# razvanmatisan/duodiff

Measured on AMD Instinct MI355X. Metric: images/sec (whole node) DuoDiff 1000-step CelebA-64, higher is better.
Workload: dtype bf16

## Files before the change

duodiff_amd/csrc/dd_internal.h:

```cpp
#pragma once
#include <hip/hip_runtime.h>
#include <stdint.h>

namespace dd {

typedef unsigned short bf16_t;

typedef __attribute__((ext_vector_type(8))) short bf16x8;
typedef __attribute__((ext_vector_type(4))) float f32x4;
typedef __attribute__((ext_vector_type(16))) float f32x16;
typedef unsigned u32x2 __attribute__((ext_vector_type(2)));
typedef unsigned u32x4 __attribute__((ext_vector_type(4)));

__device__ __forceinline__ bf16_t f2bf(float f) {
    __bf16 b = (__bf16)f;
    return __builtin_bit_cast(unsigned short, b);
}
__device__ __forceinline__ float bf2f(bf16_t b) {
    return __builtin_bit_cast(float, ((unsigned)b) << 16);
}

template <typename T> struct Elem;
template <> struct Elem<float> {
    static constexpr int kPerChunk = 4;
// ... 166 lines not shown
    const char* wimg;
    const float* bias;
    float* xres;
    const float *ln_g, *ln_b;
    bf16_t* h_out;
    bf16_t* h_frag;
    bf16_t* x_copy;
    float* partial;
    int M;
    int tok_n, tok_e, tok_l, n_main, n_extra, tiles_main, tiles_extra, groups, cpg;
};
bool rowlin_supported(int D, int K);
void rowlin_pack(int K, const float* w, unsigned short (*to_bf16)(float), unsigned short* img);
void rowlin_plan(int B, int n_patches, int extras, int seq_len, int K, RowLinArgs& a);
size_t rowlin_partial_bytes(int max_batch, int extras, int K);
hipError_t launch_rowlin(const RowLinArgs& a, hipStream_t s);
hipError_t init_rowlin_kernels();

struct EmbedArgs {
    const float* x_img;
    const float* wt;
    const float* bias;
    const float* pos;
    const float* label_emb;
    const long long* y;
    const float* t_vec;
    StepState* st;
    float* x_tok;
    int B, C, S, P, D, L, extras, num_classes, normalize, Mp;
    int generic;
    const float* ln_g = nullptr;
    const float* ln_b = nullptr;
    bf16_t* ln_frag = nullptr;
};
bool embed_ln_supported(const EmbedArgs& a);

struct ReduceLnArgs {
    float* x;
    const float* partial;
    long long slab;
    int splits, resid;
    const float* bias;
    bf16_t* copy;
    int ldo;
    const float *ln_g, *ln_b;
    bf16_t* h;
    bf16_t* frag;
    int tok_l, tok_e;
    int rows;
};
hipError_t launch_reduce_ln(const ReduceLnArgs& a, int D, hipStream_t s);
hipError_t launch_embed(const EmbedArgs& a, hipStream_t s);

struct TimeMlpArgs {
    const float *w1t, *b1, *w2t, *b2, *pos, *t_vec;
    const StepState* st;
    float* x_tok;
    int B, D, L, extras, normalize;
};
hipError_t launch_time_mlp(const TimeMlpArgs& a, hipStream_t s);

template <typename T>
hipError_t launch_layernorm(const float* x, const float* gamma, const float* beta, T* out,
                            int rows, int D, hipStream_t s);
hipError_t launch_layernorm_frag(const float* x, const float* gamma, const float* beta, bf16_t* out, bf16_t* frag, int rows, int D,
                                 int tok_l, int tok_e, hipStream_t s);
// ... 153 lines not shown
```

duodiff_amd/csrc/dev_harness.hip:

```cpp
#include "../../include/duodiff.h"
#include "../../include/duodiff_dev.h"
#include "engine_state.h"
#include "launch_args.h"

#include <cstring>
#include <vector>

using namespace dd;

extern "C" {

int dd_dev_mlp(dd_ctx* c, int M, int D, int hidden, int extras, const float* x_host, const float* w1, const float* b1, const float* w2,
               const float* b2, float* xres_host, unsigned short* out_host, const float* ln_in, const float* ln_out,
               unsigned short* ln_out_host, int iters, void* stream, float* ms_out, const float* ao_host, const float* wproj,
               const float* bproj, const float* skip_host, const float* wskip, const float* bskip, const float* wqkv,
               unsigned short* qkv_out_host) {
    const bool proj = ao_host && wproj && bproj;
    const bool skp = skip_host && wskip && bskip;
    const bool qk = wqkv && qkv_out_host;
    if (qk && (!proj || !ln_out || (hidden / 32) % 2)) return DD_ERR_INVALID;
    if (proj && (!ln_in || D % 128)) return DD_ERR_INVALID;
    if (skp && (!proj || !ln_out || !ln_out_host || (hidden / 32) % 2)) return DD_ERR_INVALID;
    if (!c || !x_host || !w1 || !b1 || !w2 || !b2 || !xres_host || M < 1 || iters < 0 || extras < 0 || (extras > 0 && M % (1 + extras))) return DD_ERR_INVALID;
    if (!mlp_fused_supported(D, hidden)) return ctx_fail(c, DD_ERR_UNSUPPORTED, "fused MLP: D in {64,128,256,512}, hidden % 64 == 0");
// ... 492 lines not shown
    const bool bf = precision == DD_PREC_BF16;
    if (!c || (!bf && precision != DD_PREC_FP32) || rows < 1 || rows > (1 << 24) || D < 64 || D % 64 || D > 4096 || !last_host || !prev_host ||
        !out_host || op < 0 || op > 2 || iters < 0)
        return DD_ERR_INVALID;
    hipStream_t s = (hipStream_t)stream;
    const size_t es = bf ? 2 : 4, n = (size_t)rows * D, n_out = ((size_t)rows + 8) * D;
    DevScope dev(c);
    const void* dL = dev.upload((const char*)last_host, n * es);
    const void* dP = dev.upload((const char*)prev_host, n * es);
    void* dO = dev.filled(n_out * es, 0xFF);
    std::vector<AffineRow> tab(3);
    memset((void*)tab.data(), 0xFF, tab.size() * sizeof(AffineRow));
    tab[1].pad1 = op; tab[1].pad2 = __builtin_bit_cast(int, w);
    const StepState st_host{1, 0.f, 0ull, 1, 0};
    const AffineRow* dT = table ? dev.upload(tab.data(), tab.size() * sizeof(AffineRow)) : nullptr;
    const StepState* dS = table ? dev.upload(&st_host, sizeof(StepState)) : nullptr;
    auto once = [&]() { return launch_cache_extrapolate(dL, dP, dO, (long long)n, bf, dS, dT, table ? -1 : op, table ? __builtin_nanf("") : w, s); };
    DEV_HIP(dev, once());
    DEV_HIP(dev, hipStreamSynchronize(s));
    dev.download(out_host, dO, n_out * es);
    DEV_HIP(dev, time_launches(s, iters, once, ms_out));
    return dev.status();
}

int dd_dev_embed(dd_ctx* c, int B, int C, int S, int P, int D, int extras, int num_classes, int normalize, int generic, const float* x_img,
                 const float* w, const float* bias, const float* pos, const float* label_emb, const long long* y, const float* t_vec,
                 float t_state, const float* ln, float* x_tok_host, unsigned short* ln_frag_host, int iters, void* stream, float* ms_out) {
    if (!c || B < 1 || C < 1 || P < 1 || S < P || S % P || D < 2 || extras < 1 || extras > 2 || !x_img || !w || !bias || !pos || !x_tok_host ||
        (extras == 2 && (!label_emb || !y || num_classes < 1)) || (ln && !ln_frag_host) || iters < 0)
        return DD_ERR_INVALID;
    const int pd = C * P * P, L = extras + (S / P) * (S / P), Mp = round_up(B * L, 256);
    if (pd > 64) return ctx_fail(c, DD_ERR_UNSUPPORTED, "embed: patch_dim <= 64");
    hipStream_t s = (hipStream_t)stream;
    const std::vector<float> wt = transposed(w, D, pd);
    const size_t n_tok = ((size_t)Mp + 8) * D;
    EmbedArgs a{};
    a.B = B; a.C = C; a.S = S; a.P = P; a.D = D; a.L = L; a.extras = extras; a.num_classes = num_classes; a.normalize = normalize; a.Mp = Mp;
    a.generic = generic;
    if (ln && !embed_ln_supported(a)) return ctx_fail(c, DD_ERR_UNSUPPORTED, "embed with norm1: the MFMA kernel at patch 4, 3 channels, embed_dim 512");
    DevScope dev(c);
    a.x_img = dev.upload(x_img, (size_t)B * C * S * S * 4);
    a.wt = dev.upload(wt.data(), wt.size() * 4);
    a.bias = dev.upload(bias, (size_t)D * 4);
    a.pos = dev.upload(pos, (size_t)L * D * 4);
    if (extras == 2) { a.label_emb = dev.upload(label_emb, (size_t)num_classes * D * 4); a.y = dev.upload(y, (size_t)B * 8); }
    if (t_vec) a.t_vec = dev.upload(t_vec, (size_t)B * 4);
    a.st = dev.alloc<StepState>(sizeof(StepState));
    a.x_tok = dev.filled<float>(n_tok * 4, 0xFF);
    if (ln) {
        a.ln_g = dev.upload(ln, (size_t)2 * D * 4); a.ln_b = a.ln_g + D;
        a.ln_frag = dev.filled<bf16_t>(n_tok * 2, 0xFF);
    }
    DEV_HIP(dev, launch_set_state_float(a.st, t_state, s));
    auto once = [&]() { return launch_embed(a, s); };
    DEV_HIP(dev, once());
    DEV_HIP(dev, hipStreamSynchronize(s));
    dev.download(x_tok_host, a.x_tok, n_tok * 4);
    if (ln) dev.download(ln_frag_host, a.ln_frag, n_tok * 2);
    DEV_HIP(dev, time_launches(s, iters, once, ms_out));
    return dev.status();
}

int dd_dev_time_mlp(dd_ctx* c, int B, int D, int L, int extras, int normalize, const float* w1, const float* b1, const float* w2,
                    const float* b2, const float* pos, const float* t_vec, float t_state, float* x_tok_host, int iters, void* stream,
                    float* ms_out) {
    if (!c || B < 1 || D < 2 || extras < 1 || L < extras || !w1 || !b1 || !w2 || !b2 || !pos || !x_tok_host || iters < 0) return DD_ERR_INVALID;
    if ((size_t)5 * D * 4 > 64 * 1024) return ctx_fail(c, DD_ERR_UNSUPPORTED, "time_mlp: 5 D floats of LDS");
    hipStream_t s = (hipStream_t)stream;
    const int H4 = 4 * D;
    const std::vector<float> w1t = transposed(w1, H4, D), w2t = transposed(w2, D, H4);
    const size_t n_tok = (size_t)B * L * D;
    DevScope dev(c);
    StepState* st = dev.alloc<StepState>(sizeof(StepState));
    float* dX = dev.upload(x_tok_host, n_tok * 4);
    const TimeMlpArgs a{dev.upload(w1t.data(), w1t.size() * 4), dev.upload(b1, (size_t)H4 * 4), dev.upload(w2t.data(), w2t.size() * 4),
// ... 421 lines not shown
```

duodiff_amd/csrc/engine_state.h:

```cpp
#pragma once
#include "../../include/duodiff.h"
#include "dd_internal.h"
#include "dev_scope.h"

#include <map>
#include <string>
#include <vector>

#define DD_HIP(c, expr)                                          \
    do {                                                         \
        hipError_t _e = (expr);                                  \
        if (_e != hipSuccess) return dd::fail_hip((c), _e, #expr);   \
    } while (0)

#pragma GCC visibility push(hidden)
namespace dd {
template <typename T>
struct DevBuf {
    T* p = nullptr;
    size_t n = 0;
    int grow(dd_ctx* c, size_t need) {
        if (n >= need) return DD_OK;
        release();
        DD_HIP(c, hipMalloc((void**)&p, need * sizeof(T)));
// ... 114 lines not shown
    bf16_t* qkv_dump = nullptr;
    bf16_t* hfrag = nullptr;
    bf16_t* aofrag = nullptr;
    std::vector<bf16_t*> skipfrags;
    float* xfrag = nullptr;
    float* ytap = nullptr;
};

struct BlockCache {
    void *last = nullptr, *prev = nullptr, *yhat = nullptr;
    int K = 0, rows = 0, b0 = 0, B = 0;
    bool has_last = false, has_prev = false;
    bool holds(int K_, int rows_, int b0_, int B_) const { return has_last && K == K_ && rows == rows_ && b0 == b0_ && B == B_; }
    void refresh(int K_, int rows_, int b0_, int B_, bool rotate) {
        has_prev = rotate && holds(K_, rows_, b0_, B_);
        K = K_; rows = rows_; b0 = b0_; B = B_; has_last = true;
    }
};

}
#pragma GCC visibility pop

struct dd_model {
    dd_ctx* ctx = nullptr;
    unsigned long long serial = 0;
    dd_config cfg{};
    int D = 0, L = 0, N = 0, extras = 0, pd = 0, pdp = 0, H = 0, hidden = 0, hid_ld = 0, half_depth = 0, Mp_max = 0;
    std::map<std::string, dd::HostParam> params;
    bool finalized = false;
    int prec = DD_PREC_BF16;
    size_t esize = 2;
    char* warena = nullptr;
    std::vector<dd::BlockW> blocks;
    const float *emb_wt = nullptr, *emb_b = nullptr, *pos = nullptr, *label = nullptr;
    const float *tm_w1t = nullptr, *tm_b1 = nullptr, *tm_w2t = nullptr, *tm_b2 = nullptr;
    dd::HeadW head{};
    int ee_type = -1, n_probe = 0;
    std::vector<dd::HeadW> heads;
    const float *probe_w = nullptr, *probe_b = nullptr;
    std::vector<dd::AttnProbeW> attn_probes;
    bool ee_conv_stride_ok = false;
    long long ee_wconv_stride = 0, ee_bconv_stride = 0;
    bool ee_batched = false;
    bool fused_mlp = false;
    bool fused_proj = false;
    bool fused_skip = false;
    bool fused_qkv = false;
    bool splitk = false;
    bool rowlin_skip = false;
    bool rowlin_proj = false;
    bool rowlin_fc2 = false;
    bool frag_ao = false;
    bool frag_skip = false;
    bool frag_x = false;
    bool fused_qa = false;
    size_t ws_bytes[2] = {0, 0};
    char* wsarena[2] = {nullptr, nullptr};
    dd::WsPtrs ws[2];
    hipGraphExec_t graph[dd::GRAPH_KINDS][2] = {};
    dd::GraphKey gkey[dd::GRAPH_KINDS][2]{};
    dd::BlockCache cache[2];
    float* ee_ws = nullptr;
    int* real_tabs = nullptr;
    int* real_counts_host = nullptr;
    hipEvent_t real_ev[2] = {nullptr, nullptr};
    bool time_fc1 = false;
    std::vector<hipEvent_t> fc1_events;
// ... 119 lines not shown
```

duodiff_amd/csrc/forward.hip:

```cpp
#include "../../include/duodiff.h"
#include "../../include/duodiff_dev.h"
#include "engine_state.h"
#include "launch_args.h"

#include <cmath>

using namespace dd;

namespace dd {
Mods perturbed(const dd_pag* p, const dd_model* late) {
    Mods mo{};
    mo.pag = p; mo.pag_late = late; mo.missing = p ? nullptr : "null dd_pag";
    return mo;
}

const char* check_threshold(const dd_x0_threshold* t) {
    if (!t) return "null dd_x0_threshold";
    if (t->mode == DD_X0_STATIC) return t->range > 0.f && std::isfinite(t->range) ? nullptr : "dd_x0_threshold: range must be positive and finite";
    if (t->mode != DD_X0_DYNAMIC) return "dd_x0_threshold: unknown mode";
    if (!(t->quantile > 0.f && t->quantile <= 1.f)) return "dd_x0_threshold: quantile outside (0, 1]";
    if (!(t->s_max >= 1.f)) return "dd_x0_threshold: s_max must be at least 1 (it may be +inf)";
    return nullptr;
}
X0Threshold kernel_threshold(const dd_x0_threshold* t, long long n) {
// ... 45 lines not shown
        if (!m->time_fc1 || kind != prof) return DD_OK;
        while (m->fc1_events.size() < m->fc1_used + 1) {
            hipEvent_t e;
            DD_HIP(c, hipEventCreate(&e));
            m->fc1_events.push_back(e);
        }
        DD_HIP(c, hipEventRecord(m->fc1_events[m->fc1_used++], s));
        return DD_OK;
    }
#define DD_TIMED(kind, expr) \
    do { if (int rc_ = mark(kind)) return rc_; DD_HIP(c, expr); if (int rc_ = mark(kind)) return rc_; } while (0)

    int tile128(int N, int K, int K1) const { return bf16 && gemm_prefers_128(m->cfg.max_batch * L, N, K, K1, c->num_cus) ? 1 : 0; }
    const T* skip_of(int bi) const { return (const T*)ws.skips[nb - 1 - bi]; }
    Handoff norm1_written() const { return Handoff{!m->fused_qa, m->fused_qa}; }

    int rowlin_then_reduce(const GemmArgs<bf16_t>& g, int resid, const char* wimg, const float* ln_g, const float* ln_b, bool frag) {
        const RowLinArgs ra = rowlin_args(g, resid, wimg, ws.mlp_partial, ln_g, ln_b, (bf16_t*)h, frag ? ws.hfrag : nullptr, B, m->N, m->extras);
        DD_TIMED(DD_PROF_ROWLIN, launch_rowlin(ra, s));
        DD_HIP(c, launch_mlp_reduce(rowlin_reduce_args(ra), D, s));
        return DD_OK;
    }
    int splitk_then_reduce_ln(GemmArgs<bf16_t> g, int resid, const float* ln_g, const float* ln_b, bool frag) {
        g.partial = ws.mlp_partial; g.splits = 2;
        DD_TIMED(DD_PROF_SPLITK, launch_gemm_splitk(g, s, ch.cus));
        DD_HIP(c, launch_reduce_ln(splitk_reduce_args(g, resid, ln_g, ln_b, (bf16_t*)h, frag ? ws.hfrag : nullptr, L, m->extras), D, s));
        return DD_OK;
    }

    int embed(const float* x_img, const float* t_vec, const int64_t* y_dev, Handoff& first) {
        EmbedArgs ea{x_img, m->emb_wt, m->emb_b, m->pos, m->label, (const long long*)y_dev, t_vec, ch.st, ws.x,
                     B, m->cfg.in_chans, m->cfg.img_size, m->cfg.patch_size, D, L, m->extras,
                     m->cfg.num_classes, m->cfg.normalize_timesteps, round_up(M, 256), (c->dev_flags & DD_DEV_GENERIC_EMBED) ? 1 : 0};
        if constexpr (bf16) {
            if (m->fused_qa && !(c->dev_flags & DD_DEV_NO_EMBED_LN) && embed_ln_supported(ea)) {
                ea.ln_g = m->blocks[0].ln1_g; ea.ln_b = m->blocks[0].ln1_b; ea.ln_frag = ws.hfrag;
                first.frag = true;
            }
        }
        DD_HIP(c, launch_embed(ea, s));
        if (m->tm_w1t) {
            TimeMlpArgs ta{m->tm_w1t, m->tm_b1, m->tm_w2t, m->tm_b2, m->pos, t_vec, ch.st, ws.x, B, D, L, m->extras, m->cfg.normalize_timesteps};
            DD_HIP(c, launch_time_mlp(ta, s));
        }
        return DD_OK;
    }

    int ee_taps(int bi, const Handoff& in, bool& side) {
        if (!ee) return DD_OK;
        const HeadW& hd = m->heads[bi];
        const float* xin = (in.skip && ws.ytap) ? ws.ytap : ws.x;
        side = bi <= m->half_depth && ch.ee_fork && c->side && s != c->side;
        hipStream_t hs = side ? c->side : s;
        if (side) {
            DD_HIP(c, hipEventRecord(c->ev_ee_fork, s));
            DD_HIP(c, hipStreamWaitEvent(c->side, c->ev_ee_fork, 0));
        }
        const int t_mul = m->ee_type == DD_EE_MLP_PER_LAYER ? 0 : m->ee_type == DD_EE_MLP_PER_TIMESTEP ? 1 : nb;
        const int add = m->ee_type == DD_EE_MLP_PER_TIMESTEP ? 0 : bi;
        bool probe_done = false;
        if (hd.wg) {
            HeadDecArgs ha{xin, hd.wg, hd.dc, ee_dec_all ? ee_dec_all + (size_t)bi * Bs * L * m->pd : ws.dec, M, m->pd, (L - m->extras) % 16 == 0 ? L : 0, m->extras};
            if (hd.wsplit) { ha.wg = hd.wsplit; ha.c = hd.dcs; ha.split = 1; }
            if (ee_srow_all && m->ee_type != DD_EE_ATTENTION_PROBE && head_dec_probe_supported(D)) {
                ha.srow = ee_srow_all + (size_t)bi * Bs * L; ha.pw_base = m->probe_w; ha.pb_base = m->probe_b; ha.st = ch.st; ha.t_mul = t_mul; ha.add = add;
                probe_done = true;
// ... 564 lines not shown
```

duodiff_amd/csrc/launch_args.h:

```cpp
#pragma once
#include "dd_internal.h"
#include "host_arena.h"

#include <cmath>
#include <vector>

namespace dd {
#pragma GCC visibility push(hidden)

inline int round_up(int v, int m) { return (v + m - 1) / m * m; }

struct TailImage {
    std::vector<unsigned short> img;
    std::vector<float> b1p;
};
inline TailImage pack_tail_image(int D, int hidden, const float* wproj, const float* w1, const float* b1, const float* w2, bool kperm, const float* wskip,
                                 const float* wqkv) {
    const MlpImage im = MlpImage::of(D, hidden, wproj != nullptr, wskip != nullptr, wqkv != nullptr);
    TailImage t{std::vector<unsigned short>(im.bytes() / 2, 0), std::vector<float>(hidden)};
    auto section = [&](size_t block) { return t.img.data() + im.at(block) / 2; };
    if (wproj) mlp_fused_pack_proj(D, wproj, host_f2bf, section(0));
    mlp_fused_pack(D, hidden, w1, b1, w2, kperm, host_f2bf, section(im.mlp), t.b1p.data());
    if (wskip) mlp_fused_pack_skip(D, wskip, host_f2bf, section(im.skip));
    if (wqkv) mlp_fused_pack_rows(D, 3 * D, wqkv, host_f2bf, section(im.qkv));
    return t;
}

inline std::vector<float> transposed(const float* w, int out, int in) {
    std::vector<float> wt((size_t)in * out);
    for (int o = 0; o < out; ++o) for (int k = 0; k < in; ++k) wt[(size_t)k * out + o] = w[(size_t)o * in + k];
    return wt;
}

struct HeadImage {
    std::vector<float> wg, dc, dcs;
    std::vector<unsigned short> wsplit;
};
inline HeadImage pack_head_image(int D, int pd, const float* wd, const float* bd, const float* ng, const float* nb, bool split) {
    HeadImage h;
    h.wg.assign((size_t)pd * D, 0.f);
    h.dc.assign(2 * (size_t)pd, 0.f);
    for (int r = 0; r < pd; ++r) {
        double acc = bd[r], wsum = 0.0;
        for (int k = 0; k < D; ++k) {
            h.wg[(size_t)r * D + k] = wd[(size_t)r * D + k] * ng[k];
            acc += (double)wd[(size_t)r * D + k] * (double)nb[k];
            wsum += (double)h.wg[(size_t)r * D + k];
        }
        h.dc[r] = (float)acc;
        h.dc[pd + r] = (float)wsum;
    }
    if (split) {
        h.wsplit = std::vector<unsigned short>((size_t)(D / 32) * ((pd + 15) / 16) * 2 * 64 * 8, 0);
        const float* c = h.dc.data();
        h.dcs.assign(c, c + 2 * (size_t)pd);
        pack_head_split(D, pd, h.wg.data(), host_f2bf, h.wsplit.data(), h.dcs.data() + pd);
    }
    return h;
}

struct AttnProbeFold {
    std::vector<float> u, wvt, w0t;
};
inline AttnProbeFold fold_attn_probe(int D, const float* q, const float* wkv, const float* w0) {
// ... 65 lines not shown
```

duodiff_amd/csrc/model.hip:

```cpp
#include "../../include/duodiff.h"
#include "../../include/duodiff_dev.h"
#include "engine_state.h"
#include "host_arena.h"
#include "launch_args.h"

#include <algorithm>
#include <atomic>
#include <cmath>
#include <cstring>
#include <map>
#include <new>
#include <string>
#include <vector>

using namespace dd;

namespace dd {
int ctx_fail(dd_ctx* c, int code, const std::string& msg) {
    if (c) c->err = msg;
    return code;
}
}

namespace {
// ... 163 lines not shown
    auto P = [&](const std::string& n) -> const std::vector<float>& { return param(m, n); };
    BlockW& w = m->blocks[bi];
    a.f32(w.ln1_g, P(p + "norm1.weight")); a.f32(w.ln1_b, P(p + "norm1.bias"));
    a.f32(w.ln2_g, P(p + "norm2.weight")); a.f32(w.ln2_b, P(p + "norm2.bias"));
    a.f32(w.proj_b, P(p + "attn.proj.bias"));
    a.f32(w.fc1_b, P(p + "mlp.fc1.bias")); a.f32(w.fc2_b, P(p + "mlp.fc2.bias"));
    a.mat(w.qkv_w, P(p + "attn.qkv.weight")); a.mat(w.proj_w, P(p + "attn.proj.weight"));
    if (m->cfg.qkv_bias) a.f32(w.qkv_b, P(p + "attn.qkv.bias"));
    a.mat(w.fc1_w, P(p + "mlp.fc1.weight")); a.mat(w.fc2_w, P(p + "mlp.fc2.weight"));
    const bool skip = bi > m->half_depth;
    if (skip) { a.f32(w.skip_b, P(p + "skip_linear.bias")); a.mat(w.skip_w, P(p + "skip_linear.weight")); }
    if (m->fused_mlp) {
        const bool with_skip = m->fused_skip && !next_skip.empty();
        const bool with_qkv = m->fused_qkv && !m->fused_qa && !next_qkv.empty() && (next_skip.empty() || with_skip);
        const TailImage t = pack_tail_image(D, hid, m->fused_proj ? P(p + "attn.proj.weight").data() : nullptr, P(p + "mlp.fc1.weight").data(),
                                            P(p + "mlp.fc1.bias").data(), P(p + "mlp.fc2.weight").data(), true,
                                            with_skip ? P(next_skip + "skip_linear.weight").data() : nullptr,
                                            with_qkv ? P(next_qkv + "attn.qkv.weight").data() : nullptr);
        std::memcpy(a.raw(w.mlp_img, t.img.size() * 2), t.img.data(), t.img.size() * 2);
        a.f32(w.mlp_b1p, t.b1p);
    }
    if (m->fused_qa)
        qkv_attention_pack(D, m->H, P(p + "attn.qkv.weight").data(), host_f2bf, (unsigned short*)a.raw(w.qa_img, (size_t)3 * D * D * 2));
    if (m->rowlin_fc2) {
        rowlin_pack(hid, P(p + "mlp.fc2.weight").data(), host_f2bf, (unsigned short*)a.raw(w.rl_img, (size_t)D * hid * 2));
        rowlin_pack(D, P(p + "attn.proj.weight").data(), host_f2bf, (unsigned short*)a.raw(w.rlp_img, (size_t)D * D * 2));
        if (skip) rowlin_pack(2 * D, P(p + "skip_linear.weight").data(), host_f2bf, (unsigned short*)a.raw(w.rls_img, (size_t)D * 2 * D * 2));
    }
}

void pack_embed(dd_model* m, Arena& a) {
    const int D = m->D, pd = m->pd;
    auto P = [&](const std::string& n) -> const std::vector<float>& { return param(m, n); };
    a.f32(m->emb_wt, transposed(P("patch_embed.proj.weight").data(), D, pd)); a.f32(m->emb_b, P("patch_embed.proj.bias")); a.f32(m->pos, P("pos_embed"));
    if (m->cfg.num_classes > 0) a.f32(m->label, P("label_emb.weight"));
    if (m->cfg.mlp_time_embed) {
        a.f32(m->tm_w1t, transposed(P("time_embed.0.weight").data(), 4 * D, D)); a.f32(m->tm_b1, P("time_embed.0.bias"));
        a.f32(m->tm_w2t, transposed(P("time_embed.2.weight").data(), D, 4 * D)); a.f32(m->tm_b2, P("time_embed.2.bias"));
    }
}

void pack_head(const dd_model* m, Arena& a, const std::string& p, HeadW& h, bool fused, bool split) {
    const int D = m->D, pd = m->pd;
    auto P = [&](const std::string& n) -> const std::vector<float>& { return param(m, n); };
    const std::vector<float>&ng = P(p + "norm.weight"), &nb = P(p + "norm.bias"), &wd = P(p + "decoder_pred.weight"), &bd = P(p + "decoder_pred.bias");
    a.f32(h.ng, ng); a.f32(h.nb, nb); a.f32(h.wdec, wd); a.f32(h.bdec, bd);
    a.f32(h.wconv, P(p + "final_layer.weight")); a.f32(h.bconv, P(p + "final_layer.bias"));
    if (!fused) return;
    const HeadImage hi = pack_head_image(D, pd, wd.data(), bd.data(), ng.data(), nb.data(), split);
    a.f32(h.wg, hi.wg); a.f32(h.dc, hi.dc);
    if (!split) return;
    std::memcpy(a.raw(h.wsplit, hi.wsplit.size() * 2), hi.wsplit.data(), hi.wsplit.size() * 2);
    a.f32(h.dcs, hi.dcs);
}

void pack_probes(dd_model* m, Arena& a) {
    const int D = m->D;
    auto P = [&](const std::string& n) -> const std::vector<float>& { return param(m, n); };
    int nt, nl;
    probe_grid(m, nt, nl);
    if (m->ee_type == DD_EE_ATTENTION_PROBE) {
        m->attn_probes.resize(nl);
        for (int layer = 0; layer < nl; ++layer) {
            const std::string pre = "matrix." + probe_key(m, layer, 0) + ".";
            const std::vector<float>&q = P(pre + "q"), &wkv = P(pre + "weight_kv.weight"), &bkv = P(pre + "weight_kv.bias"),
                                    &w0 = P(pre + "classification.0.weight");
            const AttnProbeFold f = fold_attn_probe(D, q.data(), wkv.data(), w0.data());
// ... 246 lines not shown
```

duodiff_amd/csrc/rowops.hip:

```cpp
#include "dd_internal.h"
#include "wave_prims.h"

#include <cstring>
#include <utility>
#include <vector>

#include <cstdlib>

namespace dd {
namespace {

constexpr int kEmbedTok = 8;

__global__ void __launch_bounds__(256) embed_kernel(const EmbedArgs a) {
    __shared__ float patch[kEmbedTok][64];
    const int rows_per_img_blocks = (a.L + kEmbedTok - 1) / kEmbedTok;
    const int b = blockIdx.x / rows_per_img_blocks;
    const int r0 = (blockIdx.x % rows_per_img_blocks) * kEmbedTok;
    const int tid = threadIdx.x;
    const int pd = a.C * a.P * a.P;
    const int g = a.S / a.P;
    if (blockIdx.x == 0 && tid == 0) a.st->t_final = a.st->t;

    if (b >= a.B) {
// ... 33 lines not shown
#pragma unroll
            for (int j = 0; j < kEmbedTok; ++j) acc[j] = fmaf(w, patch[j][k], acc[j]);
        }
        const float bias = a.bias[d];
#pragma unroll
        for (int j = 0; j < kEmbedTok; ++j) {
            const int row = r0 + j;
            if (row >= a.L) continue;
            float v;
            if (row >= a.extras) {
                v = acc[j] + bias;
            } else if (row == a.extras - 1) {
                const int i = d < halfd ? d : d - halfd;
                const float f = expf((-9.210340371976184f * (float)i) / (float)halfd);
                const float arg = tt * f;
                v = (d < halfd) ? cosf(arg) : (d < 2 * halfd ? sinf(arg) : 0.f);
            } else {
                long long yy = a.y[b];
                yy = yy < 0 ? 0 : (yy >= a.num_classes ? a.num_classes - 1 : yy);
                v = a.label_emb[yy * a.D + d];
            }
            a.x_tok[((long long)b * a.L + row) * a.D + d] = v + a.pos[(long long)row * a.D + d];
        }
    }
}

template <int P, int C, int LND = 0>
__global__ void __launch_bounds__(512) embed_mfma_kernel(const EmbedArgs a) {
    constexpr int PD = P * P * C, KK = PD / 4, KK4 = (KK + 3) / 4;
    static_assert(PD % 4 == 0, "k-steps of 4");
    extern __shared__ __attribute__((aligned(16))) char emb_lds[];
    f32x4* wl = reinterpret_cast<f32x4*>(emb_lds);
    const int tid = threadIdx.x, lane = tid & 63, wave = tid >> 6, n = lane & 15, kq = lane >> 4;
    const int D = a.D, S = a.S, NP = D / 32;
    const int NPY = NP / (int)gridDim.y, p0 = (int)blockIdx.y * NPY;
    const int pass = blockIdx.x * 8 + wave, b = pass >> 4, gy = pass & 15;
    const bool valid = b < a.B;
    if (blockIdx.x == 0 && tid == 0) a.st->t_final = a.st->t;

    float pv[KK];
#pragma unroll
    for (int kk = 0; kk < KK; ++kk) {
        const int k = 4 * kk + kq, c = k / (P * P), p1 = (k / P) % P, p2 = k % P;
        pv[kk] = valid ? a.x_img[(((long long)b * C + c) * S + gy * P + p1) * S + n * P + p2] : 0.f;
    }
    {
        const int items = NPY * 2 * KK4 * 64;
        constexpr int MAXI = 16;
        for (int base = 0; base < items; base += 512 * MAXI) {
            f32x4 v[MAXI];
#pragma unroll
            for (int i = 0; i < MAXI; ++i) {
                const int item = base + tid + 512 * i;
                v[i] = f32x4{0.f, 0.f, 0.f, 0.f};
                if (item < items) {
                    const int l = item & 63, kk4 = (item >> 6) % KK4, ph = (item >> 6) / KK4;
                    const int col = 16 * (ph + 2 * p0) + (l & 15);
#pragma unroll
                    for (int j = 0; j < 4; ++j) {
                        const int kk = 4 * kk4 + j;
                        if (kk < KK) v[i][j] = a.wt[(long long)(4 * kk + (l >> 4)) * D + col];
                    }
                }
            }
#pragma unroll
            for (int i = 0; i < MAXI; ++i) {
                const int item = base + tid + 512 * i;
                if (item < items) wl[item] = v[i];
            }
        }
    }
    __syncthreads();
    if (valid) {
        const long long l0 = a.extras + gy * 16 + n;
        float* xrow = a.x_tok + ((long long)b * a.L + l0) * D + 4 * kq;
        const float* prow = a.pos + l0 * D + 4 * kq;
        const float* brow = a.bias + 4 * kq;
        const f32x4* wlp = wl + lane;
        struct Quads { f32x4 pe, po, be, bo; };
        auto fetch = [&](int pp) -> Quads {
            return Quads{*reinterpret_cast<const f32x4*>(prow + 32 * pp), *reinterpret_cast<const f32x4*>(prow + 32 * pp + 16),
                         *reinterpret_cast<const f32x4*>(brow + 32 * pp), *reinterpret_cast<const f32x4*>(brow + 32 * pp + 16)};
        };
        auto pair = [&](int pp, const Quads& q) {
            f32x4 acc_e = {0.f, 0.f, 0.f, 0.f}, acc_o = {0.f, 0.f, 0.f, 0.f};
#pragma unroll
            for (int kk4 = 0; kk4 < KK4; ++kk4) {
                const f32x4 we = wlp[((2 * (pp - p0)) * KK4 + kk4) * 64], wo = wlp[((2 * (pp - p0) + 1) * KK4 + kk4) * 64];
#pragma unroll
                for (int j = 0; j < 4; ++j) {
                    if (4 * kk4 + j < KK) {
                        acc_e = __builtin_amdgcn_mfma_f32_16x16x4f32(we[j], pv[4 * kk4 + j], acc_e, 0, 0, 0);
                        acc_o = __builtin_amdgcn_mfma_f32_16x16x4f32(wo[j], pv[4 * kk4 + j], acc_o, 0, 0, 0);
                    }
                }
            }
            const f32x4 ve = (acc_e + q.be) + q.pe, vo = (acc_o + q.bo) + q.po;
            *reinterpret_cast<f32x4*>(xrow + 32 * pp) = ve;
            *reinterpret_cast<f32x4*>(xrow + 32 * pp + 16) = vo;
            return std::pair<f32x4, f32x4>{ve, vo};
        };
        Quads qa = fetch(p0), qb = qa;
        if constexpr (LND > 0) {
            constexpr int NPC = LND / 32;
            f32x4 keep[2 * NPC];
#pragma unroll
            for (int p = 0; p < NPC; p += 2) {
                qb = fetch(p + 1);
                const auto r0 = pair(p, qa);
                keep[2 * p] = r0.first; keep[2 * p + 1] = r0.second;
                qa = fetch(p + 2 < NPC ? p + 2 : p + 1);
                const auto r1 = pair(p + 1, qb);
                keep[2 * p + 2] = r1.first; keep[2 * p + 3] = r1.second;
            }
            f32x4 s4 = {0.f, 0.f, 0.f, 0.f};
#pragma unroll
            for (int t = 0; t < 2 * NPC; ++t) s4 += keep[t];
            float sum = (s4[0] + s4[1]) + (s4[2] + s4[3]);
            sum += __shfl_xor(sum, 16);
            sum += __shfl_xor(sum, 32);
            const float mean = sum / (float)LND;
            f32x4 q4 = {0.f, 0.f, 0.f, 0.f};
#pragma unroll
            for (int t = 0; t < 2 * NPC; ++t) { const f32x4 d = keep[t] - mean; q4 += d * d; }
            float q2 = (q4[0] + q4[1]) + (q4[2] + q4[3]);
            q2 += __shfl_xor(q2, 16);
            q2 += __shfl_xor(q2, 32);
            const float rstd = 1.0f / sqrtf(q2 / (float)LND + 1e-5f);
            const long long grp = (long long)b * 8 + (gy >> 1);
            bf16_t* frow = a.ln_frag + ((grp * (LND / 16)) * 64 + ((gy & 1) * 16 + n) + 32 * (kq >> 1)) * 8 + 4 * (kq & 1);
            const float* gr = a.ln_g + 4 * kq;
            const float* br = a.ln_b + 4 * kq;
#pragma unroll
            for (int t = 0; t < 2 * NPC; ++t) {
                const f32x4 gq = *reinterpret_cast<const f32x4*>(gr + 16 * t), bq = *reinterpret_cast<const f32x4*>(br + 16 * t);
                bf16_t o4[4];
#pragma unroll
                for (int e = 0; e < 4; ++e) o4[e] = f2bf((keep[t][e] - mean) * rstd * gq[e] + bq[e]);
                *reinterpret_cast<uint2*>(frow + (long long)t * 512) = *reinterpret_cast<const uint2*>(o4);
            }
        } else {
            for (int p = p0; p < p0 + NPY; p += 2) {
                qb = fetch(p + 1);
                pair(p, qa);
                qa = fetch(p + 2 < p0 + NPY ? p + 2 : p + 1);
                pair(p + 1, qb);
            }
        }
    }
    if (blockIdx.y == 0 && ((blockIdx.x * 8) & 15) == 0 && (int)(blockIdx.x * 8) / 16 < a.B) {
        const int bb = (blockIdx.x * 8) >> 4;
        const float t_raw = a.t_vec ? a.t_vec[bb] : a.st->t_model;
        const float tt = a.normalize ? t_raw / 1000.0f : t_raw;
        const int halfd = D / 2;
        for (int row = 0; row < a.extras; ++row)
            for (int d = tid; d < D; d += 512) {
                float v;
                if (row == a.extras - 1) {
                    const int i = d < halfd ? d : d - halfd;
                    const float arg = tt * expf((-9.210340371976184f * (float)i) / (float)halfd);
                    v = d < halfd ? cosf(arg) : (d < 2 * halfd ? sinf(arg) : 0.f);
                } else {
                    long long yy = a.y[bb];
                    yy = yy < 0 ? 0 : (yy >= a.num_classes ? a.num_classes - 1 : yy);
                    v = a.label_emb[yy * D + d];
                }
                a.x_tok[((long long)bb * a.L + row) * D + d] = v + a.pos[(long long)row * D + d];
            }
    }
    if (blockIdx.x == gridDim.x - 1 && blockIdx.y == 0) {
        const long long first = (long long)a.B * a.L * D, count = ((long long)a.Mp - (long long)a.B * a.L) * D;
        for (long long i = tid; i < count; i += 512) a.x_tok[first + i] = 0.f;
    }
}

__global__ void __launch_bounds__(256) time_mlp_kernel(const TimeMlpArgs a) {
    extern __shared__ float tm_lds[];
    float* e = tm_lds;
    float* hmid = tm_lds + a.D;
    const int b = blockIdx.x, tid = threadIdx.x, D = a.D, H4 = 4 * a.D, halfd = a.D / 2;
    const float t_raw = a.t_vec ? a.t_vec[b] : a.st->t_model;
    const float tt = a.normalize ? t_raw / 1000.0f : t_raw;
    for (int d = tid; d < D; d += 256) {
        const int i = d < halfd ? d : d - halfd;
        const float arg = tt * expf((-9.210340371976184f * (float)i) / (float)halfd);
        e[d] = d < halfd ? cosf(arg) : (d < 2 * halfd ? sinf(arg) : 0.f);
    }
    __syncthreads();
    for (int j = tid; j < H4; j += 256) {
        float acc = a.b1[j];
        for (int k = 0; k < D; ++k) acc = fmaf(a.w1t[(long long)k * H4 + j], e[k], acc);
        hmid[j] = acc / (1.0f + expf(-acc));
    }
    __syncthreads();
    float* row = a.x_tok + ((long long)b * a.L + a.extras - 1) * D;
    for (int d = tid; d < D; d += 256) {
        float acc = a.b2[d];
        for (int k = 0; k < H4; ++k) acc = fmaf(a.w2t[(long long)k * D + d], hmid[k], acc);
        row[d] = acc + a.pos[(long long)(a.extras - 1) * D + d];
    }
}

constexpr int kLnMaxPerLane = 16;

template <typename T>
// ... 218 lines not shown
        float a = w.bv[j];
        for (int k = 0; k < D; ++k) a = fmaf(w.wvt[(long long)k * D + j], xbar[k], a);
        ov[j] = a;
    }
    __syncthreads();
    float part = 0.f;
    for (int j = tid; j < D; j += 256) {
        float a = w.b0[j];
        for (int k = 0; k < D; ++k) a = fmaf(w.w0t[(long long)k * D + j], ov[k], a);
        hc[j] = a / (1.0f + expf(-a));
        part = fmaf(w.w2[j], hc[j], part);
    }
    part = block_reduce(part, false);
    if (tid == 0) out[b] = part + w.b2[0];
}

}

bool embed_mfma_ok(const EmbedArgs& a, size_t& lds) {
    const int pd = a.C * a.P * a.P;
    lds = (size_t)(a.D / 32) * 2 * ((pd / 4 + 3) / 4) * 1024;
    return a.S == 16 * a.P && a.D % 32 == 0 && pd % 4 == 0 && lds <= 156 * 1024 && a.L == a.extras + 256 &&
           ((a.P == 4 && a.C == 3) || (a.P == 2 && a.C == 3) || (a.P == 2 && a.C == 4));
}

bool embed_ln_supported(const EmbedArgs& a) {
    size_t lds = 0;
    return !a.generic && embed_mfma_ok(a, lds) && a.P == 4 && a.C == 3 && a.D == 512;
}

hipError_t launch_embed(const EmbedArgs& a, hipStream_t s) {
    size_t mlds = 0;
    if (!a.generic && embed_mfma_ok(a, mlds)) {
        dim3 grid((unsigned)((a.B * 16 + 7) / 8));
        if (a.ln_frag) {
            if (!embed_ln_supported(a) || !a.ln_g || !a.ln_b) return hipErrorInvalidValue;
            hipLaunchKernelGGL((embed_mfma_kernel<4, 3, 512>), grid, dim3(512), mlds, s, a);
            return hipGetLastError();
        }
        const int np = a.D / 32;
        while (grid.x * grid.y * 2 <= 256 && np % (grid.y * 4) == 0) grid.y *= 2;
        if (a.P == 4) hipLaunchKernelGGL((embed_mfma_kernel<4, 3>), grid, dim3(512), mlds, s, a);
        else if (a.C == 3) hipLaunchKernelGGL((embed_mfma_kernel<2, 3>), grid, dim3(512), mlds, s, a);
        else hipLaunchKernelGGL((embed_mfma_kernel<2, 4>), grid, dim3(512), mlds, s, a);
        return hipGetLastError();
    }
    const int per_img = (a.L + kEmbedTok - 1) / kEmbedTok;
    const long long pad_rows = (long long)a.Mp - (long long)a.B * a.L;
    const int pad_blocks = (int)((pad_rows + kEmbedTok - 1) / kEmbedTok);
    hipLaunchKernelGGL(embed_kernel, dim3(a.B * per_img + pad_blocks), dim3(256), 0, s, a);
    return hipGetLastError();
}

hipError_t launch_time_mlp(const TimeMlpArgs& a, hipStream_t s) {
    hipLaunchKernelGGL(time_mlp_kernel, dim3(a.B), dim3(256), (size_t)5 * a.D * sizeof(float), s, a);
    return hipGetLastError();
}

template <typename T>
hipError_t launch_layernorm(const float* x, const float* gamma, const float* beta, T* out, int rows,
                            int D, hipStream_t s) {
    if (D % 64 || D > 64 * kLnMaxPerLane) return hipErrorInvalidValue;
    hipLaunchKernelGGL(layernorm_kernel<T>, dim3((rows + 3) / 4), dim3(256), 0, s, x, gamma, beta, out, rows, D, (T*)nullptr, 0, 0);
    return hipGetLastError();
}
hipError_t launch_layernorm_frag(const float* x, const float* gamma, const float* beta, bf16_t* out, bf16_t* frag, int rows, int D,
                                 int tok_l, int tok_e, hipStream_t s) {
    if (D % 256 || D > 64 * kLnMaxPerLane || !frag || tok_l <= tok_e || (tok_l - tok_e) % 32 || rows % tok_l) return hipErrorInvalidValue;
    hipLaunchKernelGGL(layernorm_kernel<bf16_t>, dim3((rows + 3) / 4), dim3(256), 0, s, x, gamma, beta, out, rows, D, frag, tok_l, tok_e);
    return hipGetLastError();
// ... 326 lines not shown
```

Baseline: 49.86.

## Prepack patch-embed weights into MFMA layout and restructure embed kernel loads

```diff
diff --git a/duodiff_amd/csrc/dd_internal.h b/duodiff_amd/csrc/dd_internal.h
--- a/duodiff_amd/csrc/dd_internal.h
+++ b/duodiff_amd/csrc/dd_internal.h
@@ -222,6 +222,7 @@
     const float* ln_g = nullptr;
     const float* ln_b = nullptr;
     bf16_t* ln_frag = nullptr;
+    const float* wimg = nullptr;
 };
 bool embed_ln_supported(const EmbedArgs& a);
 
diff --git a/duodiff_amd/csrc/dev_harness.hip b/duodiff_amd/csrc/dev_harness.hip
--- a/duodiff_amd/csrc/dev_harness.hip
+++ b/duodiff_amd/csrc/dev_harness.hip
@@ -548,7 +548,7 @@
     const int pd = C * P * P, L = extras + (S / P) * (S / P), Mp = round_up(B * L, 256);
     if (pd > 64) return ctx_fail(c, DD_ERR_UNSUPPORTED, "embed: patch_dim <= 64");
     hipStream_t s = (hipStream_t)stream;
-    const std::vector<float> wt = transposed(w, D, pd);
+    const std::vector<float> wt = transposed(w, D, pd), wimg = pack_embed_image(D, pd, w);
     const size_t n_tok = ((size_t)Mp + 8) * D;
     EmbedArgs a{};
     a.B = B; a.C = C; a.S = S; a.P = P; a.D = D; a.L = L; a.extras = extras; a.num_classes = num_classes; a.normalize = normalize; a.Mp = Mp;
@@ -557,6 +557,7 @@
     DevScope dev(c);
     a.x_img = dev.upload(x_img, (size_t)B * C * S * S * 4);
     a.wt = dev.upload(wt.data(), wt.size() * 4);
+    if (!wimg.empty()) a.wimg = dev.upload(wimg.data(), wimg.size() * 4);
     a.bias = dev.upload(bias, (size_t)D * 4);
     a.pos = dev.upload(pos, (size_t)L * D * 4);
     if (extras == 2) { a.label_emb = dev.upload(label_emb, (size_t)num_classes * D * 4); a.y = dev.upload(y, (size_t)B * 8); }
diff --git a/duodiff_amd/csrc/engine_state.h b/duodiff_amd/csrc/engine_state.h
--- a/duodiff_amd/csrc/engine_state.h
+++ b/duodiff_amd/csrc/engine_state.h
@@ -170,7 +170,7 @@
     size_t esize = 2;
     char* warena = nullptr;
     std::vector<dd::BlockW> blocks;
-    const float *emb_wt = nullptr, *emb_b = nullptr, *pos = nullptr, *label = nullptr;
+    const float *emb_wt = nullptr, *emb_img = nullptr, *emb_b = nullptr, *pos = nullptr, *label = nullptr;
     const float *tm_w1t = nullptr, *tm_b1 = nullptr, *tm_w2t = nullptr, *tm_b2 = nullptr;
     dd::HeadW head{};
     int ee_type = -1, n_probe = 0;
diff --git a/duodiff_amd/csrc/forward.hip b/duodiff_amd/csrc/forward.hip
--- a/duodiff_amd/csrc/forward.hip
+++ b/duodiff_amd/csrc/forward.hip
@@ -101,6 +101,7 @@
         EmbedArgs ea{x_img, m->emb_wt, m->emb_b, m->pos, m->label, (const long long*)y_dev, t_vec, ch.st, ws.x,
                      B, m->cfg.in_chans, m->cfg.img_size, m->cfg.patch_size, D, L, m->extras,
                      m->cfg.num_classes, m->cfg.normalize_timesteps, round_up(M, 256), (c->dev_flags & DD_DEV_GENERIC_EMBED) ? 1 : 0};
+        ea.wimg = m->emb_img;
         if constexpr (bf16) {
             if (m->fused_qa && !(c->dev_flags & DD_DEV_NO_EMBED_LN) && embed_ln_supported(ea)) {
                 ea.ln_g = m->blocks[0].ln1_g; ea.ln_b = m->blocks[0].ln1_b; ea.ln_frag = ws.hfrag;
diff --git a/duodiff_amd/csrc/launch_args.h b/duodiff_amd/csrc/launch_args.h
--- a/duodiff_amd/csrc/launch_args.h
+++ b/duodiff_amd/csrc/launch_args.h
@@ -30,6 +30,21 @@
     std::vector<float> wt((size_t)in * out);
     for (int o = 0; o < out; ++o) for (int k = 0; k < in; ++k) wt[(size_t)k * out + o] = w[(size_t)o * in + k];
     return wt;
+}
+
+inline std::vector<float> pack_embed_image(int D, int pd, const float* w) {
+    if (D % 32 || pd % 4) return {};
+    const int KK = pd / 4, KK4 = (KK + 3) / 4;
+    std::vector<float> img((size_t)(D / 16) * KK4 * 64 * 4, 0.f);
+    if (img.size() * 4 > 156 * 1024) return {};
+    for (int ph = 0; ph < D / 16; ++ph)
+        for (int kk4 = 0; kk4 < KK4; ++kk4)
+            for (int l = 0; l < 64; ++l)
+                for (int j = 0; j < 4; ++j) {
+                    const int kk = 4 * kk4 + j, col = 16 * ph + (l & 15);
+                    if (kk < KK) img[(((size_t)ph * KK4 + kk4) * 64 + l) * 4 + j] = w[(size_t)col * pd + 4 * kk + (l >> 4)];
+                }
+    return img;
 }
 
 struct HeadImage {
diff --git a/duodiff_amd/csrc/model.hip b/duodiff_amd/csrc/model.hip
--- a/duodiff_amd/csrc/model.hip
+++ b/duodiff_amd/csrc/model.hip
@@ -219,7 +219,9 @@
 void pack_embed(dd_model* m, Arena& a) {
     const int D = m->D, pd = m->pd;
     auto P = [&](const std::string& n) -> const std::vector<float>& { return param(m, n); };
-    a.f32(m->emb_wt, transposed(P("patch_embed.proj.weight").data(), D, pd)); a.f32(m->emb_b, P("patch_embed.proj.bias")); a.f32(m->pos, P("pos_embed"));
+    a.f32(m->emb_wt, transposed(P("patch_embed.proj.weight").data(), D, pd));
+    if (const std::vector<float> img = pack_embed_image(D, pd, P("patch_embed.proj.weight").data()); !img.empty()) a.f32(m->emb_img, img);
+    a.f32(m->emb_b, P("patch_embed.proj.bias")); a.f32(m->pos, P("pos_embed"));
     if (m->cfg.num_classes > 0) a.f32(m->label, P("label_emb.weight"));
     if (m->cfg.mlp_time_embed) {
         a.f32(m->tm_w1t, transposed(P("time_embed.0.weight").data(), 4 * D, D)); a.f32(m->tm_b1, P("time_embed.0.bias"));
diff --git a/duodiff_amd/csrc/rowops.hip b/duodiff_amd/csrc/rowops.hip
--- a/duodiff_amd/csrc/rowops.hip
+++ b/duodiff_amd/csrc/rowops.hip
@@ -89,8 +89,8 @@
     extern __shared__ __attribute__((aligned(16))) char emb_lds[];
     f32x4* wl = reinterpret_cast<f32x4*>(emb_lds);
     const int tid = threadIdx.x, lane = tid & 63, wave = tid >> 6, n = lane & 15, kq = lane >> 4;
-    const int D = a.D, S = a.S, NP = D / 32;
-    const int NPY = NP / (int)gridDim.y, p0 = (int)blockIdx.y * NPY;
+    const int D = LND > 0 ? LND : a.D, S = a.S, NP = D / 32;
+    const int NPY = LND > 0 ? NP : NP / (int)gridDim.y, p0 = LND > 0 ? 0 : (int)blockIdx.y * NPY;
     const int pass = blockIdx.x * 8 + wave, b = pass >> 4, gy = pass & 15;
     const bool valid = b < a.B;
     if (blockIdx.x == 0 && tid == 0) a.st->t_final = a.st->t;
@@ -99,111 +99,23 @@
 #pragma unroll
     for (int kk = 0; kk < KK; ++kk) {
         const int k = 4 * kk + kq, c = k / (P * P), p1 = (k / P) % P, p2 = k % P;
-        pv[kk] = valid ? a.x_img[(((long long)b * C + c) * S + gy * P + p1) * S + n * P + p2] : 0.f;
-    }
-    {
-        const int items = NPY * 2 * KK4 * 64;
-        constexpr int MAXI = 16;
-        for (int base = 0; base < items; base += 512 * MAXI) {
-            f32x4 v[MAXI];
-#pragma unroll
-            for (int i = 0; i < MAXI; ++i) {
-                const int item = base + tid + 512 * i;
-                v[i] = f32x4{0.f, 0.f, 0.f, 0.f};
-                if (item < items) {
-                    const int l = item & 63, kk4 = (item >> 6) % KK4, ph = (item >> 6) / KK4;
-                    const int col = 16 * (ph + 2 * p0) + (l & 15);
-#pragma unroll
-                    for (int j = 0; j < 4; ++j) {
-                        const int kk = 4 * kk4 + j;
-                        if (kk < KK) v[i][j] = a.wt[(long long)(4 * kk + (l >> 4)) * D + col];
-                    }
-                }
-            }
-#pragma unroll
-            for (int i = 0; i < MAXI; ++i) {
-                const int item = base + tid + 512 * i;
-                if (item < items) wl[item] = v[i];
-            }
-        }
-    }
-    __syncthreads();
-    if (valid) {
-        const long long l0 = a.extras + gy * 16 + n;
-        float* xrow = a.x_tok + ((long long)b * a.L + l0) * D + 4 * kq;
-        const float* prow = a.pos + l0 * D + 4 * kq;
-        const float* brow = a.bias + 4 * kq;
-        const f32x4* wlp = wl + lane;
-        struct Quads { f32x4 pe, po, be, bo; };
-        auto fetch = [&](int pp) -> Quads {
-            return Quads{*reinterpret_cast<const f32x4*>(prow + 32 * pp), *reinterpret_cast<const f32x4*>(prow + 32 * pp + 16),
-                         *reinterpret_cast<const f32x4*>(brow + 32 * pp), *reinterpret_cast<const f32x4*>(brow + 32 * pp + 16)};
-        };
-        auto pair = [&](int pp, const Quads& q) {
-            f32x4 acc_e = {0.f, 0.f, 0.f, 0.f}, acc_o = {0.f, 0.f, 0.f, 0.f};
-#pragma unroll
-            for (int kk4 = 0; kk4 < KK4; ++kk4) {
-                const f32x4 we = wlp[((2 * (pp - p0)) * KK4 + kk4) * 64], wo = wlp[((2 * (pp - p0) + 1) * KK4 + kk4) * 64];
-#pragma unroll
-                for (int j = 0; j < 4; ++j) {
-                    if (4 * kk4 + j < KK) {
-                        acc_e = __builtin_amdgcn_mfma_f32_16x16x4f32(we[j], pv[4 * kk4 + j], acc_e, 0, 0, 0);
-                        acc_o = __builtin_amdgcn_mfma_f32_16x16x4f32(wo[j], pv[4 * kk4 + j], acc_o, 0, 0, 0);
-                    }
-                }
-            }
-            const f32x4 ve = (acc_e + q.be) + q.pe, vo = (acc_o + q.bo) + q.po;
-            *reinterpret_cast<f32x4*>(xrow + 32 * pp) = ve;
-            *reinterpret_cast<f32x4*>(xrow + 32 * pp + 16) = vo;
-            return std::pair<f32x4, f32x4>{ve, vo};
-        };
-        Quads qa = fetch(p0), qb = qa;
-        if constexpr (LND > 0) {
-            constexpr int NPC = LND / 32;
-            f32x4 keep[2 * NPC];
-#pragma unroll
-            for (int p = 0; p < NPC; p += 2) {
-                qb = fetch(p + 1);
-                const auto r0 = pair(p, qa);
-                keep[2 * p] = r0.first; keep[2 * p + 1] = r0.second;
-                qa = fetch(p + 2 < NPC ? p + 2 : p + 1);
-                const auto r1 = pair(p + 1, qb);
-                keep[2 * p + 2] = r1.first; keep[2 * p + 3] = r1.second;
-            }
-            f32x4 s4 = {0.f, 0.f, 0.f, 0.f};
-#pragma unroll
-            for (int t = 0; t < 2 * NPC; ++t) s4 += keep[t];
-            float sum = (s4[0] + s4[1]) + (s4[2] + s4[3]);
-            sum += __shfl_xor(sum, 16);
-            sum += __shfl_xor(sum, 32);
-            const float mean = sum / (float)LND;
-            f32x4 q4 = {0.f, 0.f, 0.f, 0.f};
-#pragma unroll
-            for (int t = 0; t < 2 * NPC; ++t) { const f32x4 d = keep[t] - mean; q4 += d * d; }
-            float q2 = (q4[0] + q4[1]) + (q4[2] + q4[3]);
-            q2 += __shfl_xor(q2, 16);
-            q2 += __shfl_xor(q2, 32);
-            const float rstd = 1.0f / sqrtf(q2 / (float)LND + 1e-5f);
-            const long long grp = (long long)b * 8 + (gy >> 1);
-            bf16_t* frow = a.ln_frag + ((grp * (LND / 16)) * 64 + ((gy & 1) * 16 + n) + 32 * (kq >> 1)) * 8 + 4 * (kq & 1);
-            const float* gr = a.ln_g + 4 * kq;
-            const float* br = a.ln_b + 4 * kq;
-#pragma unroll
-            for (int t = 0; t < 2 * NPC; ++t) {
-                const f32x4 gq = *reinterpret_cast<const f32x4*>(gr + 16 * t), bq = *reinterpret_cast<const f32x4*>(br + 16 * t);
-                bf16_t o4[4];
-#pragma unroll
-                for (int e = 0; e < 4; ++e) o4[e] = f2bf((keep[t][e] - mean) * rstd * gq[e] + bq[e]);
-                *reinterpret_cast<uint2*>(frow + (long long)t * 512) = *reinterpret_cast<const uint2*>(o4);
-            }
-        } else {
-            for (int p = p0; p < p0 + NPY; p += 2) {
-                qb = fetch(p + 1);
-                pair(p, qa);
-                qa = fetch(p + 2 < p0 + NPY ? p + 2 : p + 1);
-                pair(p + 1, qb);
-            }
-        }
+        pv[kk] = a.x_img[(((long long)(valid ? b : 0) * C + c) * S + gy * P + p1) * S + n * P + p2];
+    }
+    constexpr int MAXI = LND > 0 ? LND / 32 * 2 * KK4 * 64 / 512 : 20;
+    const int items = NPY * 2 * KK4 * 64;
+    const f32x4* wsrc = reinterpret_cast<const f32x4*>(a.wimg) + (long long)p0 * 2 * KK4 * 64;
+    f32x4 wv[MAXI], gbv = {0.f, 0.f, 0.f, 0.f};
+#pragma unroll
+    for (int i = 0; i < MAXI; ++i) {
+        const int item = tid + 512 * i;
+        wv[i] = f32x4{0.f, 0.f, 0.f, 0.f};
+        if (LND > 0 || item < items) wv[i] = wsrc[item];
+    }
+    constexpr int kLnAhead = 6;
+    f32x4 keep[LND > 0 ? LND / 16 : 1];
+    if constexpr (LND > 0) {
+        if (tid < 3 * LND / 4)
+            gbv = *reinterpret_cast<const f32x4*>(tid < LND / 4 ? a.ln_g + 4 * tid : tid < LND / 2 ? a.ln_b + 4 * (tid - LND / 4) : a.bias + 4 * (tid - LND / 2));
     }
     if (blockIdx.y == 0 && ((blockIdx.x * 8) & 15) == 0 && (int)(blockIdx.x * 8) / 16 < a.B) {
         const int bb = (blockIdx.x * 8) >> 4;
@@ -225,9 +137,100 @@
                 a.x_tok[((long long)bb * a.L + row) * D + d] = v + a.pos[(long long)row * D + d];
             }
     }
-    if (blockIdx.x == gridDim.x - 1 && blockIdx.y == 0) {
-        const long long first = (long long)a.B * a.L * D, count = ((long long)a.Mp - (long long)a.B * a.L) * D;
-        for (long long i = tid; i < count; i += 512) a.x_tok[first + i] = 0.f;
+#pragma unroll
+    for (int i = 0; i < MAXI; ++i) {
+        const int item = tid + 512 * i;
+        if (LND > 0 || item < items) wl[item] = wv[i];
+    }
+    const f32x4* gbl = wl + items;
+    if constexpr (LND > 0) {
+        if (tid < 3 * LND / 4) wl[items + tid] = gbv;
+        const float* prow = a.pos + ((long long)a.extras + gy * 16 + n) * D + 4 * kq;
+#pragma unroll
+        for (int t = 0; t < 2 * kLnAhead; ++t) keep[t] = *reinterpret_cast<const f32x4*>(prow + 16 * t);
+    }
+    __syncthreads();
+    if (valid) {
+        const long long l0 = a.extras + gy * 16 + n;
+        float* xrow = a.x_tok + ((long long)b * a.L + l0) * D + 4 * kq;
+        const float* prow = a.pos + l0 * D + 4 * kq;
+        const float* brow = a.bias + 4 * kq;
+        const f32x4* wlp = wl + lane;
+        struct Quads { f32x4 pe, po, be, bo; };
+        auto fetch = [&](int pp) -> Quads {
+            return Quads{*reinterpret_cast<const f32x4*>(prow + 32 * pp), *reinterpret_cast<const f32x4*>(prow + 32 * pp + 16),
+                         *reinterpret_cast<const f32x4*>(brow + 32 * pp), *reinterpret_cast<const f32x4*>(brow + 32 * pp + 16)};
+        };
+        auto pair = [&](int pp, const Quads& q) {
+            f32x4 acc_e = {0.f, 0.f, 0.f, 0.f}, acc_o = {0.f, 0.f, 0.f, 0.f};
+#pragma unroll
+            for (int kk4 = 0; kk4 < KK4; ++kk4) {
+                const f32x4 we = wlp[((2 * (pp - p0)) * KK4 + kk4) * 64], wo = wlp[((2 * (pp - p0) + 1) * KK4 + kk4) * 64];
+#pragma unroll
+                for (int j = 0; j < 4; ++j) {
+                    if (4 * kk4 + j < KK) {
+                        acc_e = __builtin_amdgcn_mfma_f32_16x16x4f32(we[j], pv[4 * kk4 + j], acc_e, 0, 0, 0);
+                        acc_o = __builtin_amdgcn_mfma_f32_16x16x4f32(wo[j], pv[4 * kk4 + j], acc_o, 0, 0, 0);
+                    }
+                }
+            }
+            const f32x4 ve = (acc_e + q.be) + q.pe, vo = (acc_o + q.bo) + q.po;
+            *reinterpret_cast<f32x4*>(xrow + 32 * pp) = ve;
+            *reinterpret_cast<f32x4*>(xrow + 32 * pp + 16) = vo;
+            return std::pair<f32x4, f32x4>{ve, vo};
+        };
+        if constexpr (LND > 0) {
+            constexpr int NPC = LND / 32;
+            const f32x4* bl = gbl + LND / 2 + kq;
+#pragma unroll
+            for (int p = 0; p < NPC; ++p) {
+                if (p + kLnAhead < NPC) {
+                    keep[2 * (p + kLnAhead)] = *reinterpret_cast<const f32x4*>(prow + 32 * (p + kLnAhead));
+                    keep[2 * (p + kLnAhead) + 1] = *reinterpret_cast<const f32x4*>(prow + 32 * (p + kLnAhead) + 16);
+                }
+                const auto r = pair(p, Quads{keep[2 * p], keep[2 * p + 1], bl[8 * p], bl[8 * p + 4]});
+                keep[2 * p] = r.first; keep[2 * p + 1] = r.second;
+            }
+            f32x4 s4 = {0.f, 0.f, 0.f, 0.f};
+#pragma unroll
+            for (int t = 0; t < 2 * NPC; ++t) s4 += keep[t];
+            float sum = (s4[0] + s4[1]) + (s4[2] + s4[3]);
+            sum += __shfl_xor(sum, 16);
+            sum += __shfl_xor(sum, 32);
+            const float mean = sum / (float)LND;
+            f32x4 q4 = {0.f, 0.f, 0.f, 0.f};
+#pragma unroll
+            for (int t = 0; t < 2 * NPC; ++t) { const f32x4 d = keep[t] - mean; q4 += d * d; }
+            float q2 = (q4[0] + q4[1]) + (q4[2] + q4[3]);
+            q2 += __shfl_xor(q2, 16);
+            q2 += __shfl_xor(q2, 32);
+            const float rstd = 1.0f / sqrtf(q2 / (float)LND + 1e-5f);
+            const long long grp = (long long)b * 8 + (gy >> 1);
+            bf16_t* frow = a.ln_frag + ((grp * (LND / 16)) * 64 + ((gy & 1) * 16 + n) + 32 * (kq >> 1)) * 8 + 4 * (kq & 1);
+            const f32x4* gr = gbl + kq;
+            const f32x4* br = gbl + LND / 4 + kq;
+#pragma unroll
+            for (int t = 0; t < 2 * NPC; ++t) {
+                const f32x4 gq = gr[4 * t], bq = br[4 * t];
+                bf16_t o4[4];
+#pragma unroll
+                for (int e = 0; e < 4; ++e) o4[e] = f2bf((keep[t][e] - mean) * rstd * gq[e] + bq[e]);
+                *reinterpret_cast<uint2*>(frow + (long long)t * 512) = *reinterpret_cast<const uint2*>(o4);
+            }
+        } else {
+            Quads qa = fetch(p0), qb = qa;
+            for (int p = p0; p < p0 + NPY; p += 2) {
+                qb = fetch(p + 1);
+                pair(p, qa);
+                qa = fetch(p + 2 < p0 + NPY ? p + 2 : p + 1);
+                pair(p + 1, qb);
+            }
+        }
+    }
+    if (blockIdx.y == 0) {
+        const long long count = ((long long)a.Mp - (long long)a.B * a.L) * D / 4;
+        f32x4* x4 = reinterpret_cast<f32x4*>(a.x_tok + (long long)a.B * a.L * D);
+        for (long long i = (long long)blockIdx.x * 512 + tid; i < count; i += (long long)gridDim.x * 512) x4[i] = f32x4{0.f, 0.f, 0.f, 0.f};
     }
 }
 
@@ -512,10 +515,11 @@
 hipError_t launch_embed(const EmbedArgs& a, hipStream_t s) {
     size_t mlds = 0;
     if (!a.generic && embed_mfma_ok(a, mlds)) {
+        if (!a.wimg) return hipErrorInvalidValue;
         dim3 grid((unsigned)((a.B * 16 + 7) / 8));
         if (a.ln_frag) {
             if (!embed_ln_supported(a) || !a.ln_g || !a.ln_b) return hipErrorInvalidValue;
-            hipLaunchKernelGGL((embed_mfma_kernel<4, 3, 512>), grid, dim3(512), mlds, s, a);
+            hipLaunchKernelGGL((embed_mfma_kernel<4, 3, 512>), grid, dim3(512), mlds + 3 * 512 * sizeof(float), s, a);
             return hipGetLastError();
         }
         const int np = a.D / 32;
```

Result: no change. 49.74 (-0.2%).
